# mapbox/robosat

Hardware: AMD Instinct MI355X
Metric: 512x512 tiles/sec train+predict, 1/2/4/8 MI355X; mIoU vs CPU ref (higher is better)
Workload: dtype f32; 1 GPU; rs predict ResNet50-UNet, bs=16 3x512x512 fp32 per GPU, 2 classes (BASELINE configs[1]); parallelism=tiles sharded over 1 rank(s), no collective

## Files before the change

### include/robosat_hip.h

```cpp
#ifndef ROBOSAT_HIP_H
#define ROBOSAT_HIP_H

#include <stdint.h>

#ifdef __cplusplus
extern "C" {
#endif

#define RS_EINVAL (-22)

typedef void* rs_stream_t;

typedef uint16_t rs_bf16;
#define RS_F32 0
#define RS_BF16 1

int rs_abi_version(void);

typedef struct rs_conv_desc {
  int32_t N;
  int32_t Hs, Ws;
  int32_t C1, C2;
  int32_t ups;
  int32_t kh, kw, stride, pad;
// ... 139 lines not shown

int rs_pack_phase_weight_dt(const float* w_krsc, void* out, int dtype, int Cout, int Cin, rs_stream_t stream);
int rs_pack_s2_dgrad_phase_weight_dt(const float* w_krsc, void* out, int dtype, int Cout, int Cin, rs_stream_t stream);
int rs_conv2d_fwd_phase_dt(const rs_conv_desc* d, int dtype, const void* src1, const void* src2, const void* weight_phase,
                           const float* scale, const float* shift, const void* residual, const void* relu_mask, void* out,
                           rs_stream_t stream);

int rs_conv2d_phase_wino_ok(const rs_conv_desc* d);
const char* rs_conv2d_phase_wino_name(const rs_conv_desc* d);
int rs_pack_wino_phase_weight(const float* w_phase, float* u, int Cout, int Cin, rs_stream_t stream);
int rs_conv2d_fwd_phase_wino(const rs_conv_desc* d, const float* src1, const float* src2, const float* u, float* out,
                             rs_stream_t stream);
int rs_conv2d_dgrad_phase_wino_ok(const rs_conv_desc* d);
const char* rs_conv2d_dgrad_phase_wino_name(const rs_conv_desc* d);
int rs_pack_wino_dgrad_weight(const float* wd4x4, float* u, int Cin, int Cout, rs_stream_t stream);
int rs_conv2d_dgrad_phase_wino(const rs_conv_desc* d, const float* dz, const float* u, float* out, const float* mask, float* out2,
                               const float* mask2, int csplit, rs_stream_t stream);

int rs_conv2d_wino33_ok(const rs_conv_desc* d);
const char* rs_conv2d_wino33_name(const rs_conv_desc* d);
int rs_pack_wino33_weight(const float* w_krsc, float* u, int Cout, int Cin, rs_stream_t stream);
int rs_conv2d_fwd_wino33(const rs_conv_desc* d, const float* src, const float* u, const float* scale, const float* shift, float* out,
                         rs_stream_t stream);
int rs_conv2d_wino33_head_ok(const rs_conv_desc* d, int C);
const char* rs_conv2d_wino33_head_name(void);
int rs_conv2d_fwd_wino33_head(const rs_conv_desc* d, const float* src, const float* u, const float* scale, const float* shift,
                              const float* final_w, const float* final_b, int C, int mode, const double* anchors, int overlap,
                              float* out, uint8_t* qout, rs_stream_t stream);
int rs_bottleneck_tail_f32(const float* x, const float* w3, const float* scale3, const float* shift3, const float* identity,
                           const float* w1, const float* scale1, const float* shift1, float* out, float* z, long M, int C1, int Cmid,
                           int C2, rs_stream_t stream);
int rs_conv1x1_wave_f32(const float* x, const float* w, const float* scale, const float* shift, const float* residual, int relu, float* out,
                        long M, int C1, int Cout, rs_stream_t stream);
long rs_conv2d_wino33_stats_rows(const rs_conv_desc* d);
int rs_conv2d_fwd_wino33_stats(const rs_conv_desc* d, const float* src, const float* u, float* out, float* stats, rs_stream_t stream);
int rs_conv2d_dgrad_wino33(const rs_conv_desc* d, const float* dy, const float* u, const float* mask, const uint8_t* mask_bits,
                           const float* bn_y, const float* bn_mean, const float* bn_invstd, float* out, float* stats,
                           rs_stream_t stream);

int rs_pack_dgrad_phase_weight_dt(const float* w_krsc, void* out, int dtype, int Cout, int Cin, rs_stream_t stream);
typedef struct rs_wprep_item {
  const float* w;
  rs_bf16* cast;
  rs_bf16* dgrad;
  int Cout, taps, Cin;
  int tile_begin;
} rs_wprep_item;
int rs_weight_prep_bf16(const rs_wprep_item* items_dev, int n, int total_tiles, rs_stream_t stream);
int rs_weight_prep_f32(const rs_wprep_item* items_dev, int n, int total_tiles, rs_stream_t stream);
int rs_combine_dgrad_phase_weight_dt(const float* w_dgrad, void* out, int dtype, int Cout, int Cin, rs_stream_t stream);
int rs_conv2d_fwd_split_dt(const rs_conv_desc* d, int dtype, const void* src1, const void* weight, void* out1, const void* mask1,
                           void* out2, const void* mask2, int csplit, rs_stream_t stream);
int rs_cat_split_bwd_dt(const void* dcat, void* d1, void* d2, const void* mask1, const void* mask2, int dtype, int N, int H,
                        int W, int C1, int C2, int accumulate1, rs_stream_t stream);
int rs_scatter_add_stride2_dt(const void* t, void* out, int dtype, int N, int Hs, int Ws, int Ho, int Wo, int C, rs_stream_t stream);

int rs_conv2d_dgrad_bnstats_dt(const rs_conv_desc* d, int dtype, const void* dy, const void* weight, const void* residual,
                               const void* relu_mask, const void* bn_y, const float* bn_mean, const float* bn_invstd,
                               void* out, float* stats_partial, rs_stream_t stream);
int rs_bn_bwd_from_partials_dt(const void* g, const void* y, const float* mean, const float* invstd, const float* gamma,
                               void* dy, float* dgamma, float* dbeta, const float* partial, long rows, int dtype, long M,
                               int C, void* workspace, rs_stream_t stream);
int rs_bn_apply_bits_dt(const void* y, const float* scale, const float* shift, const void* residual, void* out,
                        unsigned char* bits, int dtype, long M, int C, int relu, rs_stream_t stream);
int rs_conv2d_dgrad_bnstats_bits_dt(const rs_conv_desc* d, int dtype, const void* dy, const void* weight, const void* residual,
                                    const unsigned char* relu_mask_bits, const void* bn_y, const float* bn_mean,
// ... 63 lines not shown
```

### robosat_amd/_lib.py

```python

import ctypes
import os
from ctypes import POINTER, c_char_p, c_float, c_int, c_int32, c_long, c_void_p

import torch

_HERE = os.path.dirname(os.path.abspath(__file__))
LIB_PATH = os.environ.get("ROBOSAT_HIP_LIB") or os.path.join(_HERE, "librobosat_hip.so")

RS_EINVAL = -22
ABI_VERSION = 24
RS_F32, RS_BF16 = 0, 1
RS_TTA_IN_U8, RS_TTA_IN_F32 = 0, 1
RS_TTA_PROBS, RS_TTA_QUANTIZE, RS_TTA_ARGMAX = 0, 1, 2


class ConvDesc(ctypes.Structure):

    _fields_ = [
        ("N", c_int32), ("Hs", c_int32), ("Ws", c_int32), ("C1", c_int32), ("C2", c_int32), ("ups", c_int32),
        ("kh", c_int32), ("kw", c_int32), ("stride", c_int32), ("pad", c_int32), ("Ho", c_int32), ("Wo", c_int32),
        ("Cout", c_int32), ("relu", c_int32), ("stem", c_int32),
    ]


P = c_void_p

SIGNATURES = {
    "rs_abi_version": (c_int, []),
    "rs_conv2d_fwd": (c_int, [POINTER(ConvDesc), P, P, P, P, P, P, P, P, P]),
    "rs_conv2d_tile": (c_int, [POINTER(ConvDesc)]),
    "rs_conv2d_tile_name": (c_char_p, [c_int]),
    "rs_pack_stem_weight": (c_int, [P, P, c_int, c_int, c_int, c_int, P]),
    "rs_nchw_to_nhwc4": (c_int, [P, P, c_int, c_int, c_int, c_int, P]),
    "rs_maxpool2d_fwd": (c_int, [P, P, P, c_int, c_int, c_int, c_int, c_int, c_int, c_int, c_int, c_int, P]),
    "rs_bn_fold": (c_int, [P, P, P, P, c_float, P, P, c_int, P]),
    "rs_final_conv1x1": (c_int, [P, P, P, P, c_int, c_int, c_int, c_int, c_int, c_int, P]),
    "rs_conv2d_wgrad_workspace_bytes": (c_long, [POINTER(ConvDesc)]),
    "rs_conv2d_wgrad": (c_int, [POINTER(ConvDesc), P, P, P, P, P, P]),
    "rs_unpack_stem_weight": (c_int, [P, P, c_int, c_int, c_int, c_int, P]),
    "rs_pack_dgrad_weight": (c_int, [P, P, c_int, c_int, c_int, c_int, P]),
    "rs_bn_workspace_bytes": (c_long, [c_long, c_int]),
    "rs_bn_train_stats": (c_int, [P, c_long, c_int, c_float, c_float, P, P, P, P, P, P, P, P, P, P, P]),
    "rs_bn_apply": (c_int, [P, P, P, P, P, c_long, c_int, c_int, P]),
    "rs_bn_bwd": (c_int, [P, P, P, P, P, P, P, P, P, P, c_long, c_int, P, P]),
    "rs_maxpool2d_bwd": (c_int, [P, P, P, c_int, c_int, c_int, c_int, c_int, c_int, c_int, c_int, c_int, c_int, P]),
    "rs_upsample2x_bwd": (c_int, [P, P, P, P, P, c_int, c_int, c_int, c_int, c_int, c_int, P]),
    "rs_final_conv1x1_bwd_workspace_bytes": (c_long, [c_int, c_int]),
    "rs_final_conv1x1_bwd": (c_int, [P, P, P, P, P, P, c_int, c_int, c_int, c_int, c_int, c_int, P, P]),
    "rs_nll_loss_workspace_bytes": (c_long, []),
    "rs_nll_loss_fwd": (c_int, [P, P, P, P, P, c_int, c_int, c_int, c_int, c_int, c_float, P, P]),
    "rs_nll_loss_bwd": (c_int, [P, P, P, P, P, P, c_int, c_int, c_int, c_int, c_int, c_float, P]),
    "rs_miou_loss_workspace_bytes": (c_long, [c_int, c_int]),
    "rs_miou_loss_fwd": (c_int, [P, P, P, P, P, c_int, c_int, c_int, c_int, P, P]),
    "rs_miou_loss_bwd": (c_int, [P, P, P, P, P, P, c_int, c_int, c_int, c_int, P]),
    "rs_lovasz_workspace_bytes": (c_long, [c_int, c_int, c_int, c_int]),
    "rs_lovasz_fwd": (c_int, [P, P, P, P, c_int, c_int, c_int, c_int, P, P]),
    "rs_scale_by_scalar": (c_int, [P, P, P, c_long, P]),
    "rs_lovasz_softmax_workspace_bytes": (c_long, [c_int, c_int, c_int, c_int, c_int]),
    "rs_lovasz_softmax_fwd": (c_int, [P, P, P, P, P, c_int, c_int, c_int, c_int, c_int, c_int, P, P]),
    "rs_confusion_counts": (c_int, [P, P, P, c_int, c_int, c_int, c_int, P]),
    "rs_conv2d_fwd_bf16": (c_int, [POINTER(ConvDesc), P, P, P, P, P, P, P, P, P]),
    "rs_conv2d_tile_bf16": (c_int, [POINTER(ConvDesc)]),
    "rs_conv2d_config": (c_int, [POINTER(ConvDesc), c_int, c_int, POINTER(c_int), POINTER(c_int)]),
    "rs_conv2d_set_tuning": (c_int, [c_int, c_int]),
    "rs_set_knob": (c_int, [c_char_p, c_int]),
    "rs_get_knob": (c_int, [c_char_p, POINTER(c_int)]),
# ... 126 lines not shown
```

### robosat_amd/csrc/common.h

```cpp
#pragma once
#include <hip/hip_runtime.h>
#include <stdint.h>

#include "../../include/robosat_hip.h"

typedef float f32x4 __attribute__((ext_vector_type(4)));
typedef float f32x16 __attribute__((ext_vector_type(16)));
typedef __bf16 bf16_t;
typedef __bf16 bf16x4 __attribute__((ext_vector_type(4)));
typedef __bf16 bf16x8 __attribute__((ext_vector_type(8)));
typedef unsigned int u32x2 __attribute__((ext_vector_type(2)));
typedef unsigned int u32x4 __attribute__((ext_vector_type(4)));
typedef short s16x4 __attribute__((ext_vector_type(4)));
typedef short s16x8 __attribute__((ext_vector_type(8)));

__device__ __forceinline__ f32x4 rs_ld4(const float* p) { return *reinterpret_cast<const f32x4*>(p); }
__device__ __forceinline__ f32x4 rs_ld4(const bf16_t* p) {
  return __builtin_convertvector(*reinterpret_cast<const bf16x4*>(p), f32x4);
}
__device__ __forceinline__ void rs_st4(float* p, f32x4 v) { *reinterpret_cast<f32x4*>(p) = v; }
__device__ __forceinline__ void rs_st4(bf16_t* p, f32x4 v) {
  *reinterpret_cast<bf16x4*>(p) = __builtin_convertvector(v, bf16x4);
}
__device__ __forceinline__ float rs_ld1(const float* p) { return *p; }
// ... 147 lines not shown
#if defined(__HIP_DEVICE_COMPILE__)
  return (__umulhi(n, f.mul) + n) >> f.shift;
#else
  return (unsigned int)((((unsigned long long)n * f.mul) >> 32) + n) >> f.shift;
#endif
}

struct RsKnobs {
  int conv_tile = -1;
  int conv_rowb = 0;
  int conv_big = 1;
  int conv_min256 = 384;
  int conv_halo = 1;
  int conv_halo_min = 192;
  int conv_halo512 = -1;
  int conv1x1_ew = -1;
  int conv1x1_np = 0;
  int conv1x1_ew_bf16 = 0;
  int halo_ko = 0;
  int wgrad_f32_phase = 1;
  int wgrad_f32_dma = -1;
  int wgrad_f32_blocks = 2048;
  int wgrad_f32_wino = 1;
  int wgrad_f32_wino_blocks = 1024;
  int wgrad_f32_wino33 = 1;
  int wgrad_f32_wino33_blocks = 256;
  int wgrad_blocks = 96;
  int wgrad_blocks_phase = 1536;
  int wgrad_phase4 = 1;
  int wgrad_blocks_phase4 = 256;
  int wgrad_ring = 3;
  int lovasz_xcd = 1;
  int wino_wide = 1;
};
__attribute__((visibility("hidden"))) RsKnobs& rs_knobs();

__attribute__((visibility("hidden"))) int rs_wgrad_thin_plan(const rs_conv_desc* d, int* blocks, int* slices);
__attribute__((visibility("hidden"))) int rs_wgrad_thin_launch(const rs_conv_desc* d, const void* dy, const void* src,
                                                               float* partial, void* stream);

__attribute__((visibility("hidden"))) int rs_conv_thin_bf16_launch(int mode, const void* src, const void* wgt, const void* mask,
                                                                   void* out, int N, int Hs, int Ws, int relu, void* stream);

__attribute__((visibility("hidden"))) long rs_reduce_scratch_floats(long n, int splits);
__attribute__((visibility("hidden"))) int rs_reduce_splits(const float* ws, float* out, long n, int splits, float* scratch,
                                                           void* stream);

__attribute__((visibility("hidden"))) int rs_conv_dma_f32(const rs_conv_desc* d, const float* src1, const float* src2,
                                                          const float* weight, const float* scale, const float* shift,
                                                          const float* residual, const float* relu_mask, float* out,
                                                          void* stream);
__attribute__((visibility("hidden"))) int rs_conv_dma_tile(const rs_conv_desc* d);
```

### robosat_amd/csrc/knobs.hip

```cpp
#include <stdio.h>
#include <stdlib.h>
#include <string.h>

#include "common.h"

namespace {

struct Entry {
  const char* name;
  const char* env;
  int RsKnobs::*field;
  int lo, hi;
};

bool in_range(const Entry& e, int v) {
  if (v < e.lo || v > e.hi) return false;
  if (e.field == &RsKnobs::conv_rowb) return v == 0 || v == 64 || v == 128;
  return true;
}

const Entry kEntries[] = {
    {"conv_tile", "RS_CONV_TILE", &RsKnobs::conv_tile, -1, 9},
    {"conv_rowb", "RS_CONV_ROWB", &RsKnobs::conv_rowb, 0, 128},
    {"conv_big", "RS_CONV_BIG", &RsKnobs::conv_big, 0, 1},
    {"conv_min256", "RS_CONV_MIN256", &RsKnobs::conv_min256, 0, 1048576},
    {"conv_halo", "RS_CONV_HALO", &RsKnobs::conv_halo, 0, 1},
    {"conv_halo_min", "RS_CONV_HALO_MIN", &RsKnobs::conv_halo_min, 0, 1048576},
    {"conv_halo512", "RS_CONV_HALO512", &RsKnobs::conv_halo512, -1, 1},
    {"conv1x1_ew", "RS_CONV1X1_EW", &RsKnobs::conv1x1_ew, -1, 1},
    {"conv1x1_np", "RS_CONV1X1_NP", &RsKnobs::conv1x1_np, -1, 1},
    {"conv1x1_ew_bf16", "RS_CONV1X1_EW_BF16", &RsKnobs::conv1x1_ew_bf16, 0, 1},
    {"halo_ko", "RS_HALO_KO", &RsKnobs::halo_ko, 0, 4},
    {"wgrad_f32_phase", "RS_WGRAD_F32_PHASE", &RsKnobs::wgrad_f32_phase, 0, 1},
    {"wgrad_f32_dma", "RS_WGRAD_F32_DMA", &RsKnobs::wgrad_f32_dma, -1, 1},
    {"wgrad_f32_blocks", "RS_WGRAD_F32_BLOCKS", &RsKnobs::wgrad_f32_blocks, 1, 1048576},
    {"wgrad_f32_wino", "RS_WGRAD_F32_WINO", &RsKnobs::wgrad_f32_wino, 0, 1},
    {"wgrad_f32_wino_blocks", "RS_WGRAD_F32_WINO_BLOCKS", &RsKnobs::wgrad_f32_wino_blocks, 1, 1048576},
    {"wgrad_f32_wino33", "RS_WGRAD_F32_WINO33", &RsKnobs::wgrad_f32_wino33, 0, 1},
    {"wgrad_f32_wino33_blocks", "RS_WGRAD_F32_WINO33_BLOCKS", &RsKnobs::wgrad_f32_wino33_blocks, 1, 1048576},
    {"wgrad_blocks", "RS_WGRAD_BLOCKS", &RsKnobs::wgrad_blocks, 1, 1048576},
    {"wgrad_blocks_phase", "RS_WGRAD_BLOCKS_PHASE", &RsKnobs::wgrad_blocks_phase, 1, 1048576},
    {"wgrad_phase4", "RS_WGRAD_PHASE4", &RsKnobs::wgrad_phase4, 0, 1},
    {"wgrad_blocks_phase4", "RS_WGRAD_BLOCKS_PHASE4", &RsKnobs::wgrad_blocks_phase4, 1, 1048576},
    {"wgrad_ring", "RS_WGRAD_RING", &RsKnobs::wgrad_ring, 2, 7},
    {"lovasz_xcd", "RS_LOVASZ_XCD", &RsKnobs::lovasz_xcd, 0, 1},
    {"wino_wide", "ROBOSAT_WINO_WIDE", &RsKnobs::wino_wide, 0, 1},
};

}

RsKnobs& rs_knobs() {
  static RsKnobs k = [] {
    RsKnobs v;
    for (const Entry& e : kEntries)
      if (const char* s = getenv(e.env)) {
        const int x = atoi(s);
        if (in_range(e, x)) v.*(e.field) = x;
        else fprintf(stderr, "robosat_hip: %s=%s is outside [%d, %d]: ignored, the rule stays\n", e.env, s, e.lo, e.hi);
      }
    return v;
  }();
  return k;
}

extern "C" int rs_set_knob(const char* name, int value) {
  if (!name) return RS_EINVAL;
  for (const Entry& e : kEntries)
    if (strcmp(name, e.name) == 0) {
      if (!in_range(e, value)) return RS_EINVAL;
      rs_knobs().*(e.field) = value;
      return 0;
    }
  return RS_EINVAL;
}

extern "C" int rs_get_knob(const char* name, int* value) {
  if (!name || !value) return RS_EINVAL;
  for (const Entry& e : kEntries)
    if (strcmp(name, e.name) == 0) {
// ... 6 lines not shown
```

### robosat_amd/csrc/stem_f32.hip

```cpp
#include "lds_dma.h"

namespace {

struct StemArgs {
  const float* x;
  const float* w;
  const float* scale;
  const float* shift;
  float* out;
  int N, H, W, Ho, Wo, relu;
  int tpr;
  int ntile;
#ifdef RS_STEM_TRACE
  long long* trace;
#endif
};

constexpr int SBM = 128, SBN = 64;
constexpr int SCOLS = 2 * SBM + 6;
constexpr int XI = 132;
constexpr int LDO = SBN + 4;

template <int CIN>
struct Geom {
  static constexpr int PS = CIN == 3 ? 3 : 5;
  static constexpr int ROWF = 2 * XI * PS;
  static constexpr int STRIPF = 7 * ROWF;
  static constexpr int PAIR = 7 * CIN;
  static constexpr int NPAIR = 3 * PAIR;
  static constexpr int NEO = 3 * CIN;
  static constexpr int NSTEP = NPAIR + NEO + CIN;
  static constexpr int WF = NSTEP * 2 * SBN;
  static constexpr int STAGEF = SBM * LDO;
  static constexpr int REGION = STRIPF > STAGEF ? STRIPF : STAGEF;
  static constexpr int ZEROF = SBM * PS + 8;
  static constexpr int LDSF = WF + REGION + ZEROF;
};

struct Tap {
  int r, s, c;
};
template <int CIN>
__host__ __device__ constexpr Tap stem_tap(int t, int h) {
  using G = Geom<CIN>;
  if (t < G::NPAIR) return Tap{2 * (t / G::PAIR) + h, (t % G::PAIR) / CIN, t % CIN};
  const int u = t - G::NPAIR;
  return Tap{6, 2 * (u / CIN) + h, u % CIN};
}
template <int CIN>
__host__ __device__ constexpr int stem_imm(int t) {
  using G = Geom<CIN>;
  const Tap k = stem_tap<CIN>(t, 0);
  return ((k.r * 2 + (k.s & 1)) * XI + (k.s >> 1)) * G::PS + k.c;
}

template <int CIN>
__global__ __launch_bounds__(256, CIN == 3 ? 2 : 1) void stem_conv_f32(const StemArgs p) {
  using G = Geom<CIN>;
  constexpr int PS = G::PS;
  constexpr int NPF = (7 * SCOLS + 255) / 256;
  static_assert(G::LDSF * 4 <= (CIN == 3 ? 80 : 160) * 1024, "LDS");

  __shared__ __attribute__((aligned(16))) float lds[G::LDSF];
  float* const wl = lds;
  float* const strip = lds + G::WF;
  float* const zline = lds + G::WF + G::REGION;

  const int tid = threadIdx.x;
  const int lane = tid & 63;
  const int wave = tid >> 6;
  const int wm = wave >> 1, wn = wave & 1;
  const int li = lane & 31, lh = lane >> 5;

#ifdef RS_STEM_TRACE
  if (tid == 0) p.trace[((long)blockIdx.x * 64 + 63) * 8 + 0] = (long long)__builtin_amdgcn_s_memtime();
#endif
  const int t0 = (int)((long)blockIdx.x * p.ntile / gridDim.x);
  const int t1 = (int)((long)(blockIdx.x + 1) * p.ntile / gridDim.x);
  if (t0 >= t1) return;

  {
    constexpr int NW4 = SBN * 7 * 8 / 256;
    f32x4 wv[NW4];
#pragma unroll
    for (int k = 0; k < NW4; ++k) wv[k] = *reinterpret_cast<const f32x4*>(p.w + (tid + 256 * k) * 4);
#pragma unroll
    for (int k = 0; k < NW4; ++k) {
      const int e = tid + 256 * k;
      const int s_ = e & 7, r = (e >> 3) % 7, co = e / 56;
      int t, h;
      if (r < 6) {
        t = (r >> 1) * G::PAIR + s_ * CIN, h = r & 1;
        if (s_ == 7) continue;
      } else if (s_ < 6) {
        t = G::NPAIR + (s_ >> 1) * CIN, h = s_ & 1;
      } else {
        t = G::NPAIR + G::NEO, h = s_ & 1;
      }
#pragma unroll
      for (int c = 0; c < CIN; ++c) wl[((t + c) * 2 + h) * SBN + co] = wv[k][c];
    }
  }
  for (int e = tid; e < G::ZEROF; e += 256) zline[e] = 0.f;

  f32x4 pf[NPF];
  int pdst[NPF];
  int prow[NPF], pcol[NPF], prel[NPF];
#pragma unroll
  for (int q = 0; q < NPF; ++q) {
    const int e = tid + 256 * q;
    const int r = e / SCOLS, j = e - r * SCOLS;
    const bool in = e < 7 * SCOLS;
// ... 14 lines not shown
    const __amdgpu_buffer_rsrc_t rs = rs_dma_rsrc<0x7FFFFFF0u>(p.x + n * img, live ? img * 4 : 0);
    const int iy0 = 2 * oy - 3, ix0 = 2 * tx * SBM - 3;
    const int base = (iy0 * p.W + ix0) * 16;
#pragma unroll
    for (int q = 0; q < NPF; ++q) {
      const bool ok = (unsigned)(iy0 + prow[q]) < (unsigned)p.H && (unsigned)(ix0 + pcol[q]) < (unsigned)p.W;
      pf[q] = __builtin_bit_cast(f32x4, __builtin_amdgcn_raw_buffer_load_b128(rs, ok ? base + prel[q] : -1, 0, 0));
    }
  };
  auto put = [&]() __attribute__((always_inline)) {
#pragma unroll
    for (int q = 0; q < NPF; ++q) {
      if (pdst[q] >= 0) {
        float* d = strip + pdst[q];
        d[0] = pf[q][0];
        d[1] = pf[q][1];
        d[2] = pf[q][2];
        if (CIN == 4) d[3] = pf[q][3];
      }
    }
  };

  const int apix = (wm * 64 + li) * PS;
  const float* const A1 = strip + apix + lh * G::ROWF;
  const float* const A2 = strip + apix + lh * (XI * PS);
  constexpr int IMM6 = ((6 * 2 + 0) * XI + 3) * PS;
  const float* const A3 = lh ? zline + apix - IMM6 : strip + apix;
  const float* const B = wl + lh * SBN + wn * 32 + li;

  const int ecol = (tid & 15) * 4, erow = tid >> 4;
  f32x4 sc = {1.f, 1.f, 1.f, 1.f}, sh = {0.f, 0.f, 0.f, 0.f};
  if (p.scale) sc = *reinterpret_cast<const f32x4*>(p.scale + ecol);
  if (p.shift) sh = *reinterpret_cast<const f32x4*>(p.shift + ecol);

#ifdef RS_STEM_TRACE
#define STAMP(k) do { if (tid == 0) p.trace[((long)blockIdx.x * 64 + (tile - t0)) * 8 + (k)] = (long long)__builtin_amdgcn_s_memtime(); } while (0)
#else
#define STAMP(k)
#endif
#ifdef RS_STEM_TRACE
  if (tid == 0) p.trace[((long)blockIdx.x * 64 + 63) * 8 + 1] = (long long)__builtin_amdgcn_s_memtime();
#endif
  fetch(cn, coy, ctx, true);
  put();
  for (int tile = t0; tile < t1; ++tile) {
    STAMP(0);
    __syncthreads();
    STAMP(1);
    int nn = cn, noy = coy, ntx = ctx + 1;
    if (ntx == p.tpr) {
      ntx = 0;
      if (++noy == p.Ho) noy = 0, ++nn;
    }
    fetch(nn, noy, ntx, tile + 1 < t1);
    STAMP(2);

    f32x16 acc0, acc1;
#pragma unroll
    for (int r = 0; r < 16; ++r) acc0[r] = 0.f, acc1[r] = 0.f;
    constexpr int DEPTH = 3;
    float fb[DEPTH], fa0[DEPTH], fa1[DEPTH];
    auto frag = [&](int t) __attribute__((always_inline)) {
      const float* A = t < G::NPAIR ? A1 : (t < G::NPAIR + G::NEO ? A2 : A3);
      const int imm = stem_imm<CIN>(t);
      fb[t % DEPTH] = B[t * 2 * SBN];
      fa0[t % DEPTH] = A[imm];
      fa1[t % DEPTH] = A[imm + 32 * PS];
    };
#pragma unroll
    for (int t = 0; t < DEPTH; ++t) frag(t);
#pragma unroll
    for (int t = 0; t < G::NSTEP; ++t) {
      const float b = fb[t % DEPTH], a0 = fa0[t % DEPTH], a1 = fa1[t % DEPTH];
      __builtin_amdgcn_sched_barrier(0);
      acc0 = __builtin_amdgcn_mfma_f32_32x32x2f32(b, a0, acc0, 0, 0, 0);
      if (t + DEPTH < G::NSTEP) frag(t + DEPTH);
      acc1 = __builtin_amdgcn_mfma_f32_32x32x2f32(b, a1, acc1, 0, 0, 0);
      __builtin_amdgcn_sched_barrier(0);
    }
    STAMP(3);
    __syncthreads();
    STAMP(4);

    {
      const int prow = wm * 64 + li;
      const int ccol = wn * 32 + 4 * lh;
#pragma unroll
      for (int g = 0; g < 4; ++g) {
        *reinterpret_cast<f32x4*>(&strip[prow * LDO + ccol + 8 * g]) = f32x4{acc0[4 * g], acc0[4 * g + 1], acc0[4 * g + 2], acc0[4 * g + 3]};
        *reinterpret_cast<f32x4*>(&strip[(prow + 32) * LDO + ccol + 8 * g]) = f32x4{acc1[4 * g], acc1[4 * g + 1], acc1[4 * g + 2], acc1[4 * g + 3]};
      }
    }
    __syncthreads();
    f32x4 ov[SBM / 16];
#pragma unroll
    for (int i = 0; i < SBM / 16; ++i) ov[i] = *reinterpret_cast<const f32x4*>(&strip[(erow + 16 * i) * LDO + ecol]);
    __syncthreads();
    STAMP(5);
    put();
    STAMP(6);
    {
      const int ox0 = ctx * SBM;
      const int live = p.Wo - ox0 < SBM ? p.Wo - ox0 : SBM;
      float* const orow = p.out + (((long)cn * p.Ho + coy) * p.Wo + ox0) * SBN + ecol;
#pragma unroll
      for (int i = 0; i < SBM / 16; ++i) {
        const int row = erow + 16 * i;
        f32x4 v = ov[i];
#pragma unroll
        for (int e = 0; e < 4; ++e) v[e] = v[e] * sc[e] + sh[e];
        if (p.relu) {
#pragma unroll
          for (int e = 0; e < 4; ++e) v[e] = fmaxf(v[e], 0.f);
        }
        if (row < live) *reinterpret_cast<f32x4*>(orow + (long)row * SBN) = v;
      }
    }
    STAMP(7);
    cn = nn, coy = noy, ctx = ntx;
  }
#ifdef RS_STEM_TRACE
  if (tid == 0) p.trace[((long)blockIdx.x * 64 + 63) * 8 + 2] = (long long)__builtin_amdgcn_s_memtime();
#endif
}

}

__attribute__((visibility("hidden"))) int rs_stem_f32_launch(const rs_conv_desc* d, int bands, const float* x, const float* w,
                                                             const float* scale, const float* shift, float* out, void* stream) {
  if (d->kh != 7 || d->kw != 7 || d->stride != 2 || d->pad != 3 || d->Cout != SBN || d->C1 != 4) return RS_EINVAL;
  if (d->Ho != (d->Hs + 1) / 2 || d->Wo != (d->Ws + 1) / 2) return RS_EINVAL;
  if ((long)d->Hs * d->Ws * 16 >= (1L << 31)) return RS_EINVAL;
  StemArgs a;
  a.x = x, a.w = w, a.scale = scale, a.shift = shift, a.out = out;
  a.N = d->N, a.H = d->Hs, a.W = d->Ws, a.Ho = d->Ho, a.Wo = d->Wo, a.relu = d->relu;
  a.tpr = rs_cdiv(d->Wo, SBM);
  const long ntile = (long)d->N * d->Ho * a.tpr;
  if (ntile <= 0 || ntile >= (1L << 31)) return RS_EINVAL;
  a.ntile = (int)ntile;
  const int cus = rs_cu_count();
  const long want = bands == 3 ? 2L * cus : cus;
  const int grid = (int)(ntile < want ? ntile : want);
  if (bands == 3)
    stem_conv_f32<3><<<grid, 256, 0, (hipStream_t)stream>>>(a);
  else
    stem_conv_f32<4><<<grid, 256, 0, (hipStream_t)stream>>>(a);
  return RS_LAUNCH_RESULT();
}

#ifdef RS_STEM_TRACE
extern "C" int rs_stem_f32_trace(int N, int H, int W, const float* x, const float* w, float* out, long long* trace, int grid) {
  StemArgs a;
  a.x = x, a.w = w, a.scale = nullptr, a.shift = nullptr, a.out = out;
  a.N = N, a.H = H, a.W = W, a.Ho = H / 2, a.Wo = W / 2, a.relu = 1;
  a.tpr = rs_cdiv(a.Wo, SBM);
  a.ntile = N * a.Ho * a.tpr;
  a.trace = trace;
  stem_conv_f32<3><<<grid, 256, 0, 0>>>(a);
  return RS_LAUNCH_RESULT();
}
#endif
```

### robosat_amd/ops.py

```python

import ctypes
import os

import torch

from . import _lib
from ._lib import RS_BF16, RS_F32, ConvDesc, check

BF16 = torch.bfloat16


def _dt(t):

    dtype = getattr(t, "dtype", t)
    if dtype == torch.float32:
        return RS_F32
    if dtype == torch.bfloat16:
        return RS_BF16
    raise TypeError("robosat_amd: activations are fp32 or bf16, got {}".format(dtype))


def _esize(t):

    return 2 if getattr(t, "dtype", t) == BF16 else 4


def _dev(t, name, dtype=torch.float32):
    if t is None:
        return None
    if not t.is_cuda:
        raise RuntimeError("robosat_amd: `{}` is on {} -- the hot path only runs on the MI355X (no CPU fallback)".format(name, t.device))
    if t.dtype != dtype:
        raise TypeError("robosat_amd: `{}` must be {}, got {}".format(name, dtype, t.dtype))
    if not t.is_contiguous():
        raise ValueError("robosat_amd: `{}` must be contiguous".format(name))
    return ctypes.c_void_p(t.data_ptr())


def _stream():
    return ctypes.c_void_p(torch.cuda.current_stream().cuda_stream)


def _call(name, *args):

    rc = getattr(_lib.lib(), name)(*args)
    if rc:
        check(rc, name)


SWITCHES = {
    "ROBOSAT_WINOGRAD": "fp32 Winograd forward forms (DecoderBlock, stride-1 3x3); off: the generic phase / implicit-GEMM kernels",
    "ROBOSAT_WINO_DGRAD": "Winograd data gradient of the fp32 DecoderBlock; off: the 4x4 / stride-2 kernel",
    "ROBOSAT_WINO33_STATS": "train-mode fp32 conv3x3 -> BatchNorm front half in the Winograd form; off: conv2d_bnstats",
    "ROBOSAT_WINO33_BWD": "Winograd data gradient of the fp32 stride-1 3x3 convolutions; off: the generic kernel",
    "ROBOSAT_FUSED_HEAD": "dec5 + self.final in one launch; off: two launches",
    "ROBOSAT_TAIL_FUSE": "layer1's fused Bottleneck tail and its wave 1x1 kernel; off: the generic 1x1 convolutions",
    "ROBOSAT_S2_DGRAD": "stride-2 data gradients in compact form (3x3: phase form, 1x1: scatter-add); off: zero-insertion convolutions",
    "ROBOSAT_S2_DGRAD_3X3": "the 3x3 half of ROBOSAT_S2_DGRAD alone",
    "ROBOSAT_WGRAD_STREAM": "weight gradients on a side stream; off: serial backward (clean per-kernel timings)",
}


def switch(name):

    if name not in SWITCHES:
        raise KeyError("robosat_amd: unknown switch {!r}: one of {}".format(name, ", ".join(SWITCHES)))
    return os.environ.get(name, "1") != "0"


PROFILE = None


def _start():

    if PROFILE is None:
        return None
    ev = torch.cuda.Event(enable_timing=True), torch.cuda.Event(enable_timing=True)
    ev[0].record()
    return ev


def _stop(ev):
    ev[1].record()


def _record(ev, name, flops, shape, nbytes, executed=None):

    PROFILE.append((name, flops, shape, ev[0], ev[1], nbytes, flops if executed is None else executed))
# ... 587 lines not shown
        self.weights = list(weights_krsc)
        self.cast = [torch.empty(w.shape, device=dev, dtype=BF16) if dtype == BF16 else None for w in self.weights]
        self.dgrad = [torch.empty((w.shape[3], w.shape[1], w.shape[2], w.shape[0]), device=dev, dtype=dtype) if want_dgrad else None
                      for w in self.weights]
        items = (_WPrepItem * len(self.weights))()
        tiles = 0
        for i, w in enumerate(self.weights):
            cout, kh, kw, cin = w.shape
            items[i] = _WPrepItem(_dev(w, "w").value, _dev(self.cast[i], "cast", BF16).value if dtype == BF16 else None,
                                  _dev(self.dgrad[i], "dgrad", dtype).value if want_dgrad else None, cout, kh * kw, cin, tiles)
            tiles += kh * kw * ((cin + 31) // 32) * ((cout + 31) // 32)
        self.tiles = tiles
        self.table = torch.frombuffer(bytearray(bytes(items)), dtype=torch.uint8).to(dev)
        self.ptrs = tuple(w.data_ptr() for w in self.weights)

    def run(self):
        _call("rs_weight_prep_bf16" if self.dtype == BF16 else "rs_weight_prep_f32", _dev(self.table, "items", torch.uint8),
              len(self.weights), self.tiles, _stream())


def pack_stem_weight(w_krsc, dtype=torch.float32):

    cout, kh, kw, cin = w_krsc.shape
    out = torch.empty((cout, kh, 8, 4), device=w_krsc.device, dtype=dtype)
    _call("rs_pack_stem_weight_bf16" if dtype == BF16 else "rs_pack_stem_weight", _dev(w_krsc, "w"), _dev(out, "out", dtype), cout, kh, kw,
          cin, _stream())
    return out


def nchw_to_nhwc4(x, dtype=torch.float32):
    n, c, h, w = x.shape
    out = torch.empty((n, h, w, 4), device=x.device, dtype=dtype)
    _call("rs_nchw_to_nhwc4_bf16" if dtype == BF16 else "rs_nchw_to_nhwc4", _dev(x, "x"), _dev(out, "out", dtype), n, c, h, w, _stream())
    return out


def stem_conv_bf16(x4, w_packed, scale=None, shift=None, relu=False):

    n, h, w, _ = x4.shape
    out = torch.empty((n, h // 2, w // 2, 64), device=x4.device, dtype=BF16)
    ev = _start()
    _call("rs_stem_conv_fwd_bf16", _dev(x4, "x4", BF16), _dev(w_packed, "w", BF16), _dev(scale, "scale"), _dev(shift, "shift"),
          _dev(out, "out", BF16), n, h, w, int(relu), _stream())
    if ev:
        _stop(ev)
        flops = 2.0 * n * 64 * 3 * 49 * (h // 2) * (w // 2)
        _record(ev, "stem_conv_bf16", flops, (3, 64, 7, 2, 0, h // 2, w // 2), 2 * (x4.numel() + out.numel()))
    return out


def wgrad_kernel_name(d, form=None):

    lib = _lib.lib()
    if form is None:
        form = lib.rs_conv2d_wgrad_bf16_form(ctypes.byref(d))
    if form == 1:
        return "conv_wgrad_thin_bf16<{}{}>".format(min(d.C1, 128), ",ups" if d.ups else "")
    t = lib.rs_conv2d_wgrad_bf16_tile(ctypes.byref(d))
    if t <= 0:
        raise ValueError("rs_conv2d_wgrad_bf16_tile: invalid arguments")
    tile = "{}x{}".format(t >> 16, t & 255) + ("+{}x{}".format(t >> 16, (t >> 8) & 255) if (t >> 8) & 255 else "")
    phase = "" if form != 2 else ("phase4," if (t >> 16, t & 255) == (128, 128) and get_knob("wgrad_phase4") else "phase,")
    return "conv_wgrad_bf16<{}{}>".format(phase, tile)


def stem_conv_wgrad_bf16(dy, x4):
# ... 639 lines not shown
```

### robosat_amd/unet.py

```python

import math
import os
import warnings

import torch
import torch.nn as nn

from . import ops

_RESNET50_FILE = "resnet50-19c8e357.pth"


class _Conv(nn.Module):

    def __init__(self, cin, cout, k, stride=1, padding=0, bias=False, init="default"):
        super().__init__()
        self.cin, self.cout, self.k, self.stride, self.padding = cin, cout, k, stride, padding
        w = torch.empty(cout, cin, k, k).contiguous(memory_format=torch.channels_last)
        fan_in, fan_out = cin * k * k, cout * k * k
        if init == "resnet":
            nn.init.normal_(w, 0.0, math.sqrt(2.0 / fan_out))
        else:
            nn.init.uniform_(w, -1.0 / math.sqrt(fan_in), 1.0 / math.sqrt(fan_in))
        self.weight = nn.Parameter(w)
# ... 8 lines not shown
        w = w if w.is_contiguous() else w.contiguous()
        if dtype == torch.float32:
            return w
        key = (self.weight.data_ptr(), self.weight._version, _GENERATION[0])
        c = getattr(self, "_bf16", None)
        if c is None or c[0] != key:
            c = (key, ops.cast_bf16(w))
            self._bf16 = c
        return c[1]

    def dgrad_weight(self, dtype=torch.float32):

        c = getattr(self, "_dgrad" if dtype == torch.bfloat16 else "_dgrad_f32", None)
        if c is not None and c[0] == (self.weight.data_ptr(), self.weight._version, _GENERATION[0]):
            return c[1]
        return ops.pack_dgrad_weight(self.krsc(), dtype)

    def phase(self, dtype=torch.float32):

        key = (self.weight.data_ptr(), self.weight._version, _GENERATION[0], dtype)
        c = getattr(self, "_phase", None)
        if c is None or c[0] != key:
            c = (key, ops.pack_phase_weight(self.krsc(), dtype))
            self._phase = c
        return c[1]

    def phase_wino(self):

        key = (self.weight.data_ptr(), self.weight._version, _GENERATION[0])
        c = getattr(self, "_phase_wino", None)
        if c is None or c[0] != key:
            c = (key, ops.pack_wino_phase_weight(self.phase(torch.float32)))
            self._phase_wino = c
        return c[1]

    def wino33(self):

        key = (self.weight.data_ptr(), self.weight._version, _GENERATION[0])
        c = getattr(self, "_wino33", None)
        if c is None or c[0] != key:
            c = (key, ops.pack_wino33_weight(self.krsc()))
            self._wino33 = c
        return c[1]

    def dgrad_wino33(self):

        key = (self.weight.data_ptr(), self.weight._version, _GENERATION[0])
        c = getattr(self, "_dgrad_wino33", None)
        if c is None or c[0] != key:
            c = (key, ops.pack_wino33_weight(self.dgrad_weight(torch.float32)))
            self._dgrad_wino33 = c
        return c[1]

    def dgrad_s2_phase(self, dtype=torch.float32, wino=False):

        key = (self.weight.data_ptr(), self.weight._version, _GENERATION[0], dtype, wino)
        c = getattr(self, "_dgrad_s2_phase", None)
        if c is None or c[0] != key:
            pack = ops.pack_s2_dgrad_phase_weight(self.krsc(), dtype)
            c = (key, ops.pack_wino_phase_weight(pack) if wino else pack)
            self._dgrad_s2_phase = c
        return c[1]

    def dgrad_phase(self, dtype=torch.float32):

        key = (self.weight.data_ptr(), self.weight._version, _GENERATION[0], dtype)
# ... 358 lines not shown
        mean, std = list(mean)[:self.in_channels], list(std)[:self.in_channels]
        if tta != "none":
            op_list = ops.tta_ops(tta, images_u8.size(1), images_u8.size(2))

            def run(u8):
                x4 = ops.tta_fan_out_u8(u8, mean, std, op_list, self.compute_dtype)
                return ops.tta_merge(self._forward_eval(None, softmax=True, x4=x4), op_list, "argmax")
        else:
            op_list = [0]

            def run(u8):
                x4 = ops.u8_to_nhwc4_norm(u8, mean, std)
                if self.compute_dtype == torch.bfloat16:
                    x4 = x4.to(torch.bfloat16)
                return self._forward_eval(None, softmax=False, x4=x4, argmax=True)

        images_u8 = images_u8.contiguous()
        if self._want_graph(images_u8, len(op_list)):
            return self._graph_replay(("classes", tuple(mean), tuple(std), tta), run, images_u8)
        return run(images_u8)

    def _forward_eval(self, x, softmax, x4=None, quantize_overlap=None, argmax=False):
        r = self.resnet
        dt = self.compute_dtype
        if x4 is None:
            if not x.is_cuda:
                raise RuntimeError("robosat_amd.UNet runs on the MI355X only (got a {} tensor); there is no CPU fallback".format(x.device))
            assert x.size(1) == self.in_channels
            x = x.detach().float().contiguous()
            x4 = ops.nchw_to_nhwc4(x, dt)
        h = x4
        sc, sh = r.bn1.folded()
        if dt == torch.bfloat16:
            h = ops.stem_conv_bf16(h, ops.pack_stem_weight(r.conv1.krsc(), dt), scale=sc, shift=sh, relu=True)
        else:
            h = ops.conv2d(h, ops.pack_stem_weight(r.conv1.krsc()), stride=2, pad=3, scale=sc, shift=sh, relu=True, stem=7,
                           bands=self.in_channels)
        h = ops.maxpool2d(h, 3, 2, 1)

        enc = []
        for layer in self._blocks():
            blocks = list(layer)
            ahead = None
            for bi, blk in enumerate(blocks):
                if ahead is None:
                    sc, sh = blk.bn1.folded()
                    o = ops.conv2d(h, blk.conv1.krsc(dt), scale=sc, shift=sh, relu=True)
                else:
                    o, ahead = ahead, None
                sc, sh = blk.bn2.folded()
                o = conv3x3_eval(blk.conv2, o, dt, scale=sc, shift=sh)
                if blk.downsample is not None:
                    sc, sh = blk.downsample[1].folded()
                    dw = blk.downsample[0].krsc(dt)
                    if blk.stride == 1 and ops.conv1x1_wave_ok(h, dw):
                        idt = ops.conv1x1_wave(h, dw, sc, sh)
                    else:
                        idt = ops.conv2d(h, dw, stride=blk.stride, scale=sc, shift=sh)
                else:
                    idt = h
                sc, sh = blk.bn3.folded()
                nxt = blocks[bi + 1] if bi + 1 < len(blocks) else None
                if (nxt is not None and nxt.conv1.k == 1 and nxt.conv1.stride == 1 and dt == torch.float32
                        and ops.bottleneck_tail_ok(o, blk.conv3.krsc(dt), nxt.conv1.krsc(dt))):
                    sc1, sh1 = nxt.bn1.folded()
                    h, ahead = ops.bottleneck_tail(o, blk.conv3.krsc(dt), sc, sh, idt, nxt.conv1.krsc(dt), sc1, sh1)
                else:
                    h = ops.conv2d(o, blk.conv3.krsc(dt), scale=sc, shift=sh, residual=idt, relu=True)
            enc.append(h)
        enc1, enc2, enc3, enc4 = enc

# ... 21 lines not shown
```

Baseline: 1638 tiles/s.

## Fuse maxpool into fp32 eval stem conv epilogue and cache packed stem weights

Adds a POOL variant of the fp32 stem 7x7 conv kernel that performs the 3x3/2 maxpool in its epilogue. Blocks are assigned pairs of output rows, and a carried row handles the pooling window overlap, so the full-resolution stem activation is never written to or read back from memory. It also caches the packed stem weight on the conv module instead of repacking it on every forward call. The fused path is used only when the batch is large enough (units >= 4x grid). Its cost is extra register pressure and a recomputed boundary row at the start of each block.

```diff
diff --git a/include/robosat_hip.h b/include/robosat_hip.h
--- a/include/robosat_hip.h
+++ b/include/robosat_hip.h
@@ -195,6 +195,9 @@
                            int C2, rs_stream_t stream);
 int rs_conv1x1_wave_f32(const float* x, const float* w, const float* scale, const float* shift, const float* residual, int relu, float* out,
                         long M, int C1, int Cout, rs_stream_t stream);
+int rs_stem_pool_f32_ok(int N, int H, int W, int bands);
+int rs_stem_pool_f32(const float* x, const float* w_packed, const float* scale, const float* shift, float* out, int N, int H, int W,
+                     int bands, int relu, rs_stream_t stream);
 long rs_conv2d_wino33_stats_rows(const rs_conv_desc* d);
 int rs_conv2d_fwd_wino33_stats(const rs_conv_desc* d, const float* src, const float* u, float* out, float* stats, rs_stream_t stream);
 int rs_conv2d_dgrad_wino33(const rs_conv_desc* d, const float* dy, const float* u, const float* mask, const uint8_t* mask_bits,
diff --git a/robosat_amd/_lib.py b/robosat_amd/_lib.py
--- a/robosat_amd/_lib.py
+++ b/robosat_amd/_lib.py
@@ -33,6 +33,8 @@
     "rs_conv2d_tile_name": (c_char_p, [c_int]),
     "rs_pack_stem_weight": (c_int, [P, P, c_int, c_int, c_int, c_int, P]),
     "rs_nchw_to_nhwc4": (c_int, [P, P, c_int, c_int, c_int, c_int, P]),
+    "rs_stem_pool_f32_ok": (c_int, [c_int, c_int, c_int, c_int]),
+    "rs_stem_pool_f32": (c_int, [P, P, P, P, P, c_int, c_int, c_int, c_int, c_int, P]),
     "rs_maxpool2d_fwd": (c_int, [P, P, P, c_int, c_int, c_int, c_int, c_int, c_int, c_int, c_int, c_int, P]),
     "rs_bn_fold": (c_int, [P, P, P, P, c_float, P, P, c_int, P]),
     "rs_final_conv1x1": (c_int, [P, P, P, P, c_int, c_int, c_int, c_int, c_int, c_int, P]),
diff --git a/robosat_amd/csrc/common.h b/robosat_amd/csrc/common.h
--- a/robosat_amd/csrc/common.h
+++ b/robosat_amd/csrc/common.h
@@ -203,6 +203,7 @@
   int wgrad_ring = 3;
   int lovasz_xcd = 1;
   int wino_wide = 1;
+  int stem_pool_blocks = 0;
 };
 __attribute__((visibility("hidden"))) RsKnobs& rs_knobs();
 
diff --git a/robosat_amd/csrc/knobs.hip b/robosat_amd/csrc/knobs.hip
--- a/robosat_amd/csrc/knobs.hip
+++ b/robosat_amd/csrc/knobs.hip
@@ -45,6 +45,7 @@
     {"wgrad_ring", "RS_WGRAD_RING", &RsKnobs::wgrad_ring, 2, 7},
     {"lovasz_xcd", "RS_LOVASZ_XCD", &RsKnobs::lovasz_xcd, 0, 1},
     {"wino_wide", "ROBOSAT_WINO_WIDE", &RsKnobs::wino_wide, 0, 1},
+    {"stem_pool_blocks", "RS_STEM_POOL_BLOCKS", &RsKnobs::stem_pool_blocks, 0, 1048576},
 };
 
 }
diff --git a/robosat_amd/csrc/stem_f32.hip b/robosat_amd/csrc/stem_f32.hip
--- a/robosat_amd/csrc/stem_f32.hip
+++ b/robosat_amd/csrc/stem_f32.hip
@@ -11,6 +11,7 @@
   int N, H, W, Ho, Wo, relu;
   int tpr;
   int ntile;
+  int nunit;
 #ifdef RS_STEM_TRACE
   long long* trace;
 #endif
@@ -54,7 +55,9 @@
   return ((k.r * 2 + (k.s & 1)) * XI + (k.s >> 1)) * G::PS + k.c;
 }
 
-template <int CIN>
+constexpr int PTPR = 2;
+
+template <int CIN, bool POOL = false>
 __global__ __launch_bounds__(256, CIN == 3 ? 2 : 1) void stem_conv_f32(const StemArgs p) {
   using G = Geom<CIN>;
   constexpr int PS = G::PS;
@@ -75,9 +78,18 @@
 #ifdef RS_STEM_TRACE
   if (tid == 0) p.trace[((long)blockIdx.x * 64 + 63) * 8 + 0] = (long long)__builtin_amdgcn_s_memtime();
 #endif
-  const int t0 = (int)((long)blockIdx.x * p.ntile / gridDim.x);
-  const int t1 = (int)((long)(blockIdx.x + 1) * p.ntile / gridDim.x);
-  if (t0 >= t1) return;
+  int t0, t1;
+  if constexpr (POOL) {
+    const int u0 = (int)((long)blockIdx.x * p.nunit / gridDim.x);
+    const int u1 = (int)((long)(blockIdx.x + 1) * p.nunit / gridDim.x);
+    if (u0 >= u1) return;
+    t0 = (2 * u0 - (u0 % (p.Ho >> 1) != 0)) * p.tpr;
+    t1 = 2 * u1 * p.tpr;
+  } else {
+    t0 = (int)((long)blockIdx.x * p.ntile / gridDim.x);
+    t1 = (int)((long)(blockIdx.x + 1) * p.ntile / gridDim.x);
+    if (t0 >= t1) return;
+  }
 
   {
     constexpr int NW4 = SBN * 7 * 8 / 256;
@@ -158,6 +170,25 @@
   f32x4 sc = {1.f, 1.f, 1.f, 1.f}, sh = {0.f, 0.f, 0.f, 0.f};
   if (p.scale) sc = *reinterpret_cast<const f32x4*>(p.scale + ecol);
   if (p.shift) sh = *reinterpret_cast<const f32x4*>(p.shift + ecol);
+  auto affine = [&](f32x4 v) __attribute__((always_inline)) {
+#pragma unroll
+    for (int e = 0; e < 4; ++e) v[e] = v[e] * sc[e] + sh[e];
+    if (p.relu) {
+#pragma unroll
+      for (int e = 0; e < 4; ++e) v[e] = fmaxf(v[e], 0.f);
+    }
+    return v;
+  };
+  auto max4 = [](f32x4 a, const f32x4 b) __attribute__((always_inline)) {
+#pragma unroll
+    for (int e = 0; e < 4; ++e) a[e] = fmaxf(a[e], b[e]);
+    return a;
+  };
+  f32x4 vmax[PTPR][4], carry = {0.f, 0.f, 0.f, 0.f};
+#pragma unroll
+  for (int k = 0; k < PTPR; ++k)
+#pragma unroll
+    for (int j = 0; j < 4; ++j) vmax[k][j] = carry;
 
 #ifdef RS_STEM_TRACE
 #define STAMP(k) do { if (tid == 0) p.trace[((long)blockIdx.x * 64 + (tile - t0)) * 8 + (k)] = (long long)__builtin_amdgcn_s_memtime(); } while (0)
@@ -218,27 +249,62 @@
       }
     }
     __syncthreads();
-    f32x4 ov[SBM / 16];
-#pragma unroll
-    for (int i = 0; i < SBM / 16; ++i) ov[i] = *reinterpret_cast<const f32x4*>(&strip[(erow + 16 * i) * LDO + ecol]);
-    __syncthreads();
-    STAMP(5);
-    put();
-    STAMP(6);
-    {
+    if constexpr (POOL) {
+      f32x4 cv[9], last;
+#pragma unroll
+      for (int k = 0; k < 9; ++k) cv[k] = *reinterpret_cast<const f32x4*>(&strip[(erow || k ? 8 * erow - 1 + k : 0) * LDO + ecol]);
+      last = *reinterpret_cast<const f32x4*>(&strip[(SBM - 1) * LDO + ecol]);
+      __syncthreads();
+      STAMP(5);
+      put();
+      STAMP(6);
+#pragma unroll
+      for (int k = 0; k < 9; ++k) cv[k] = affine(cv[k]);
+      if (erow == 0) cv[0] = ctx > 0 ? carry : cv[1];
+      carry = affine(last);
+      f32x4 hm[4];
+#pragma unroll
+      for (int j = 0; j < 4; ++j) hm[j] = max4(max4(cv[2 * j], cv[2 * j + 1]), cv[2 * j + 2]);
+      if (coy == 0 || tile - t0 < p.tpr) {
+#pragma unroll
+        for (int j = 0; j < 4; ++j) vmax[0][j] = hm[j];
+      } else if (!(coy & 1)) {
+#pragma unroll
+        for (int j = 0; j < 4; ++j) vmax[0][j] = max4(vmax[0][j], hm[j]);
+      } else {
+        const int wp = p.Wo >> 1, px0 = ctx * (SBM / 2) + 4 * erow;
+        float* const orow = p.out + (((long)cn * (p.Ho >> 1) + (coy >> 1)) * wp + px0) * SBN + ecol;
+#pragma unroll
+        for (int j = 0; j < 4; ++j) {
+          const f32x4 v = max4(vmax[0][j], hm[j]);
+          vmax[0][j] = hm[j];
+          if (px0 + j < wp) *reinterpret_cast<f32x4*>(orow + j * SBN) = v;
+        }
+      }
+      if (p.tpr == PTPR) {
+#pragma unroll
+        for (int j = 0; j < 4; ++j) {
+          const f32x4 t = vmax[0][j];
+          vmax[0][j] = vmax[1][j];
+          vmax[1][j] = t;
+        }
+      }
+      rs_lds_writes_done();
+    } else {
+      f32x4 ov[SBM / 16];
+#pragma unroll
+      for (int i = 0; i < SBM / 16; ++i) ov[i] = *reinterpret_cast<const f32x4*>(&strip[(erow + 16 * i) * LDO + ecol]);
+      __syncthreads();
+      STAMP(5);
+      put();
+      STAMP(6);
       const int ox0 = ctx * SBM;
       const int live = p.Wo - ox0 < SBM ? p.Wo - ox0 : SBM;
       float* const orow = p.out + (((long)cn * p.Ho + coy) * p.Wo + ox0) * SBN + ecol;
 #pragma unroll
       for (int i = 0; i < SBM / 16; ++i) {
         const int row = erow + 16 * i;
-        f32x4 v = ov[i];
-#pragma unroll
-        for (int e = 0; e < 4; ++e) v[e] = v[e] * sc[e] + sh[e];
-        if (p.relu) {
-#pragma unroll
-          for (int e = 0; e < 4; ++e) v[e] = fmaxf(v[e], 0.f);
-        }
+        const f32x4 v = affine(ov[i]);
         if (row < live) *reinterpret_cast<f32x4*>(orow + (long)row * SBN) = v;
       }
     }
@@ -264,6 +330,7 @@
   const long ntile = (long)d->N * d->Ho * a.tpr;
   if (ntile <= 0 || ntile >= (1L << 31)) return RS_EINVAL;
   a.ntile = (int)ntile;
+  a.nunit = 0;
   const int cus = rs_cu_count();
   const long want = bands == 3 ? 2L * cus : cus;
   const int grid = (int)(ntile < want ? ntile : want);
@@ -274,6 +341,48 @@
   return RS_LAUNCH_RESULT();
 }
 
+namespace {
+
+int stem_pool_grid(long units, int bands) {
+  const int cus = rs_cu_count();
+  long want = bands == 3 ? 2L * cus : cus;
+  const int cap = rs_knobs().stem_pool_blocks;
+  if (cap > 0 && cap < want) want = cap;
+  return (int)(units < want ? units : want);
+}
+
+bool stem_pool_geometry(int N, int H, int W) {
+  if (N <= 0 || H < 4 || W < 4 || H % 4 || W % 4) return false;
+  if (W / 2 > PTPR * SBM) return false;
+  if ((long)H * W * 16 >= (1L << 31)) return false;
+  return (long)N * (H / 2) * rs_cdiv(W / 2, SBM) < (1L << 31);
+}
+
+}
+
+extern "C" int rs_stem_pool_f32_ok(int N, int H, int W, int bands) {
+  if (!stem_pool_geometry(N, H, W) || bands < 1 || bands > 4) return 0;
+  const long units = (long)N * (H / 4);
+  return units >= 4L * stem_pool_grid(units, bands) ? 1 : 2;
+}
+
+extern "C" int rs_stem_pool_f32(const float* x, const float* w_packed, const float* scale, const float* shift, float* out, int N, int H,
+                                int W, int bands, int relu, rs_stream_t stream) {
+  if (!x || !w_packed || !out || bands < 1 || bands > 4 || !stem_pool_geometry(N, H, W)) return RS_EINVAL;
+  StemArgs a;
+  a.x = x, a.w = w_packed, a.scale = scale, a.shift = shift, a.out = out;
+  a.N = N, a.H = H, a.W = W, a.Ho = H / 2, a.Wo = W / 2, a.relu = relu;
+  a.tpr = rs_cdiv(a.Wo, SBM);
+  a.ntile = N * a.Ho * a.tpr;
+  a.nunit = N * (a.Ho / 2);
+  const int grid = stem_pool_grid(a.nunit, bands);
+  if (bands == 3)
+    stem_conv_f32<3, true><<<grid, 256, 0, (hipStream_t)stream>>>(a);
+  else
+    stem_conv_f32<4, true><<<grid, 256, 0, (hipStream_t)stream>>>(a);
+  return RS_LAUNCH_RESULT();
+}
+
 #ifdef RS_STEM_TRACE
 extern "C" int rs_stem_f32_trace(int N, int H, int W, const float* x, const float* w, float* out, long long* trace, int grid) {
   StemArgs a;
@@ -281,6 +390,7 @@
   a.N = N, a.H = H, a.W = W, a.Ho = H / 2, a.Wo = W / 2, a.relu = 1;
   a.tpr = rs_cdiv(a.Wo, SBM);
   a.ntile = N * a.Ho * a.tpr;
+  a.nunit = 0;
   a.trace = trace;
   stem_conv_f32<3><<<grid, 256, 0, 0>>>(a);
   return RS_LAUNCH_RESULT();
diff --git a/robosat_amd/ops.py b/robosat_amd/ops.py
--- a/robosat_amd/ops.py
+++ b/robosat_amd/ops.py
@@ -54,6 +54,7 @@
     "ROBOSAT_WINO33_STATS": "train-mode fp32 conv3x3 -> BatchNorm front half in the Winograd form; off: conv2d_bnstats",
     "ROBOSAT_WINO33_BWD": "Winograd data gradient of the fp32 stride-1 3x3 convolutions; off: the generic kernel",
     "ROBOSAT_FUSED_HEAD": "dec5 + self.final in one launch; off: two launches",
+    "ROBOSAT_STEM_POOL": "fp32 eval stem with resnet.maxpool in its epilogue (large batches); off: stem, then maxpool2d",
     "ROBOSAT_TAIL_FUSE": "layer1's fused Bottleneck tail and its wave 1x1 kernel; off: the generic 1x1 convolutions",
     "ROBOSAT_S2_DGRAD": "stride-2 data gradients in compact form (3x3: phase form, 1x1: scatter-add); off: zero-insertion convolutions",
     "ROBOSAT_S2_DGRAD_3X3": "the 3x3 half of ROBOSAT_S2_DGRAD alone",
@@ -707,6 +708,28 @@
     n, c, h, w = x.shape
     out = torch.empty((n, h, w, 4), device=x.device, dtype=dtype)
     _call("rs_nchw_to_nhwc4_bf16" if dtype == BF16 else "rs_nchw_to_nhwc4", _dev(x, "x"), _dev(out, "out", dtype), n, c, h, w, _stream())
+    return out
+
+
+def stem_conv_pool_ok(x4, bands=4, force=False):
+
+    if x4.dtype != torch.float32 or not switch("ROBOSAT_STEM_POOL"):
+        return False
+    n, h, w, _ = x4.shape
+    return _lib.lib().rs_stem_pool_f32_ok(n, h, w, bands) in ((1, 2) if force else (1,))
+
+
+def stem_conv_pool(x4, w_packed, scale=None, shift=None, relu=True, bands=4):
+
+    n, h, w, _ = x4.shape
+    out = torch.empty((n, h // 4, w // 4, 64), device=x4.device, dtype=torch.float32)
+    ev = _start()
+    _call("rs_stem_pool_f32", _dev(x4, "x4"), _dev(w_packed, "w"), _dev(scale, "scale"), _dev(shift, "shift"), _dev(out, "out"), n, h, w,
+          bands, int(relu), _stream())
+    if ev:
+        _stop(ev)
+        _record(ev, "stem_conv_f32<128x64>", 2.0 * n * 64 * 3 * 49 * (h // 2) * (w // 2), (3, 64, 7, 2, 0, h // 2, w // 2),
+                4 * (x4.numel() + w_packed.numel() + out.numel()))
     return out
 
 
diff --git a/robosat_amd/unet.py b/robosat_amd/unet.py
--- a/robosat_amd/unet.py
+++ b/robosat_amd/unet.py
@@ -64,6 +64,15 @@
         if c is None or c[0] != key:
             c = (key, ops.pack_wino_phase_weight(self.phase(torch.float32)))
             self._phase_wino = c
+        return c[1]
+
+    def stem_pack(self, dtype=torch.float32):
+
+        key = (self.weight.data_ptr(), self.weight._version, _GENERATION[0], dtype)
+        c = getattr(self, "_stem_pack", None)
+        if c is None or c[0] != key:
+            c = (key, ops.pack_stem_weight(self.krsc(), dtype))
+            self._stem_pack = c
         return c[1]
 
     def wino33(self):
@@ -488,11 +497,12 @@
         h = x4
         sc, sh = r.bn1.folded()
         if dt == torch.bfloat16:
-            h = ops.stem_conv_bf16(h, ops.pack_stem_weight(r.conv1.krsc(), dt), scale=sc, shift=sh, relu=True)
+            h = ops.maxpool2d(ops.stem_conv_bf16(h, r.conv1.stem_pack(dt), scale=sc, shift=sh, relu=True), 3, 2, 1)
+        elif ops.stem_conv_pool_ok(h, self.in_channels):
+            h = ops.stem_conv_pool(h, r.conv1.stem_pack(), scale=sc, shift=sh, relu=True, bands=self.in_channels)
         else:
-            h = ops.conv2d(h, ops.pack_stem_weight(r.conv1.krsc()), stride=2, pad=3, scale=sc, shift=sh, relu=True, stem=7,
-                           bands=self.in_channels)
-        h = ops.maxpool2d(h, 3, 2, 1)
+            h = ops.maxpool2d(ops.conv2d(h, r.conv1.stem_pack(), stride=2, pad=3, scale=sc, shift=sh, relu=True, stem=7,
+                                         bands=self.in_channels), 3, 2, 1)
 
         enc = []
         for layer in self._blocks():
```

Result: no change. 1651 tiles/s (median of 6 runs) (+0.8%).
